# hrdkjain/GenIcoNet

Hardware: AMD Instinct MI355X
Metric: meshes/sec training throughput, ico2ico I5 batch=36 (higher is better)
Workload: dtype f32; 1 GPU; ico2ico AE training, I5, batch 36 per GPU (BASELINE configs[1]); per_gpu_batch=36, global_batch=36, subdivisions=5, parallelism=dp1

## Files before the change

geniconet_amd/csrc/icn_api.cpp:

```cpp
#include <hip/hip_runtime.h>

#include <algorithm>
#include <cstdio>
#include <cstdlib>
#include <cstring>
#include <map>
#include <mutex>
#include <stdexcept>
#include <string>
#include <tuple>
#include <vector>

#include "../../include/icn.h"
#include "icn_geometry.h"
#include "icn_launch.h"
#include "icn_streamk.h"

namespace {

thread_local std::string g_err;

int fail(const std::string& msg) {
    g_err = msg;
    return -1;
// ... 25 lines not shown
    int32_t* code = nullptr;
    int32_t* slots = nullptr;
    int n_slots = 0, E = 1;
};
DevDma upload_dma(const std::vector<int32_t>& idx, int E, int P) {
    icn::DmaTable h;
    icn::build_dma_table(idx, E, P, h);
    DevDma d;
    d.code = upload(h.code);
    d.slots = upload(h.slots);
    d.n_slots = h.n_slots;
    d.E = E;
    return d;
}
struct ConvTables {
    int Pin = 0, Pout = 0, n_in = 0, n_out = 0, E = 1;
    int32_t* fwd = nullptr;
    int32_t* bwd = nullptr;
    int32_t* bwd1 = nullptr;
    int nv = 0, nvp = 0;
    int32_t* vidx = nullptr;
    int32_t* vorder = nullptr;
    uint32_t* vmask32 = nullptr;
    int32_t* vq = nullptr;
    int32_t* perm = nullptr;
    int32_t* bwd_perm = nullptr;
    uint32_t* mask32 = nullptr;
    std::vector<uint32_t> mask32_h;
    int key = 0;
    DevDma d_fwd, d_bwd, d_bwd1, d_virt, d_bwdp;
    int32_t* w7_rows = nullptr;
    uint16_t* w7_pos = nullptr;
    int w7_U = 0;
};
struct UpTables {
    int Pc = 0, Pf = 0, Wf = 0, Wb = 0;
    int32_t *idx_f = nullptr, *idx_b = nullptr;
    float *coef_f = nullptr, *coef_b = nullptr;
};

struct UpconvDev {
    int Pc = 0, Pf = 0, n_slots = 0, E = 1, nseg = 0;
    int seg_cnt[icn::UPCONV_MAX_SEG] = {}, seg_off[icn::UPCONV_MAX_SEG] = {};
    uint32_t seg_mask[icn::UPCONV_MAX_SEG] = {};
    int32_t *pix = nullptr, *code = nullptr, *slot_idx = nullptr;
    float *alpha = nullptr, *slot_coef = nullptr;
};

struct EllSplitDev {
    int W = 0, n_ovf = 0, W_ovf = 0;
    int32_t *idx = nullptr, *ovf_rows = nullptr, *ovf_idx = nullptr;
    float *coef = nullptr, *ovf_coef = nullptr;
};
EllSplitDev upload_ell_split(const icn::Ell& e, int W_main) {
    EllSplitDev d;
    const int W = e.width;
    d.W = W_main;
    d.W_ovf = std::max(W - W_main, 0);
    std::vector<int32_t> idx((size_t)e.rows * W_main, icn::IDX_ZERO), ovf_rows, ovf_idx;
    std::vector<float> coef((size_t)e.rows * W_main, 0.f), ovf_coef;
    for (int r = 0; r < e.rows; ++r) {
        for (int k = 0; k < std::min(W, W_main); ++k) {
            idx[(size_t)r * W_main + k] = e.idx[(size_t)r * W + k];
            coef[(size_t)r * W_main + k] = e.coef[(size_t)r * W + k];
        }
        if (W > W_main && e.idx[(size_t)r * W + W_main] != icn::IDX_ZERO) {
            ovf_rows.push_back(r);
            for (int k = W_main; k < W; ++k) {
                ovf_idx.push_back(e.idx[(size_t)r * W + k]);
                ovf_coef.push_back(e.coef[(size_t)r * W + k]);
            }
        }
    }
    d.n_ovf = (int)ovf_rows.size();
    d.idx = upload(idx);
    d.coef = upload(coef);
    d.ovf_rows = upload(ovf_rows);
    d.ovf_idx = upload(ovf_idx);
    d.ovf_coef = upload(ovf_coef);
    return d;
}

struct PatchHost { std::vector<int32_t> prow; std::vector<uint16_t> plocal; int npatch = 0, umax = 0, gridW = 0; };
bool build_patches(const std::vector<int32_t>& idx, int width_in, int width, int H, int W, int ph, int pw, PatchHost& out) {
    out = PatchHost{};
    if (H % ph != 0 || W % pw != 0 || (long)H * W * width_in != (long)idx.size()) return false;
    const int pr_n = H / ph, pc_n = W / pw;
    out.npatch = pr_n * pc_n;
    out.gridW = W;
    out.plocal.assign((size_t)H * W * width, 0xFFFFu);
    std::vector<std::vector<int32_t>> lists(out.npatch);
    for (int p = 0; p < out.npatch; ++p) {
        std::vector<int32_t>& u = lists[p];
        for (int i = 0; i < ph; ++i)
            for (int j = 0; j < pw; ++j) {
                const size_t r = (size_t)((p / pc_n) * ph + i) * W + (p % pc_n) * pw + j;
                for (int k = 0; k < width; ++k) {
                    const int32_t v = idx[r * width_in + k];
                    if (v >= 0) u.push_back(v);
                }
            }
        std::sort(u.begin(), u.end());
        u.erase(std::unique(u.begin(), u.end()), u.end());
        out.umax = std::max(out.umax, (int)u.size());
    }
    out.umax = (out.umax + 31) / 32 * 32;
    if (out.umax == 0 || out.umax >= 0xFFFF) return false;
    out.prow.assign((size_t)out.npatch * out.umax, -1);
    for (int p = 0; p < out.npatch; ++p) {
        const std::vector<int32_t>& u = lists[p];
        std::copy(u.begin(), u.end(), out.prow.begin() + (size_t)p * out.umax);
        for (int i = 0; i < ph; ++i)
            for (int j = 0; j < pw; ++j) {
                const size_t r = (size_t)((p / pc_n) * ph + i) * W + (p % pc_n) * pw + j;
                for (int k = 0; k < width; ++k) {
                    const int32_t v = idx[r * width_in + k];
                    if (v >= 0) out.plocal[r * width + k] = (uint16_t)(std::lower_bound(u.begin(), u.end(), v) - u.begin());
                }
            }
    }
    return true;
}
struct PatchDev { int32_t* prow = nullptr; uint16_t* plocal = nullptr; int npatch = 0, umax = 0, gridW = 0; };
PatchDev upload_patches(const PatchHost& h) {
    PatchDev d;
    if (getenv("ICN_VERBOSE")) fprintf(stderr, "icn: patch table: %d patches, %d rows per list, grid width %d\n", h.npatch, h.umax, h.gridW);
    d.prow = upload(h.prow);
    d.plocal = upload(h.plocal);
    d.npatch = h.npatch; d.umax = h.umax; d.gridW = h.gridW;
    return d;
}

struct UpconvBwdDev {
    int Pc = 0, Pf = 0;
    PatchDev sc_patch, ga_patch;
    EllSplitDev gather, scatter;
    int32_t* iota = nullptr;
    int32_t* px_srcs = nullptr;
    int32_t* px_cls = nullptr;
    float* cls_coef = nullptr;
    int n_cls = 0;
};

std::mutex g_mu;
std::map<std::tuple<int, int, int>, UpconvDev> g_upconv;
std::map<std::tuple<int, int, int>, UpconvBwdDev> g_upconv_bwd;
std::map<std::tuple<int, int, int, int>, ConvTables> g_conv;
std::map<std::tuple<int, int, int>, UpTables> g_up;

static int wgrad7_union_rows(int stride) {
    if (stride != 1) return 112;
    static const int u1 = [] {
        const char* e = getenv("ICN_W7_U");
        return e ? atoi(e) : 64;
    }();
    if (u1 != 56 && u1 != 64)
        throw std::invalid_argument("icn: ICN_W7_U must be 56 or 64 (the instantiations of k_wgrad7 at stride 1), got " + std::to_string(u1));
    return u1;
}

ConvTables make_conv_tables(int r_in, int stride, int mode) {
    ConvTables t;
    t.n_in = 1 << r_in;
    t.n_out = t.n_in / stride;
    t.Pin = icn::pixels(r_in);
    t.Pout = 10 * t.n_out * t.n_out;
    std::vector<int32_t> fwd, bwd, perm;
    std::vector<uint8_t> mask;
    icn::build_conv_fwd(r_in, stride, mode, fwd);
    t.E = icn::build_conv_bwd(r_in, stride, mode, bwd);
    t.fwd = upload(fwd);
    t.bwd = upload(bwd);
    t.d_fwd = upload_dma(fwd, 1, t.Pout);
    t.d_bwd = upload_dma(bwd, t.E, t.Pin);
    {
        icn::DmaTable h;
        icn::build_dma_table(fwd, 1, t.Pout, h);
        icn::Wg7Table w7;
        if (icn::build_wgrad7(h, t.Pout, wgrad7_union_rows(stride), w7)) {
            t.w7_rows = upload(w7.urow);
            t.w7_pos = upload(w7.upos);
            t.w7_U = w7.U;
        }
    }
    std::vector<int32_t> primary;
    icn::VirtualRows vr;
    icn::split_conv_bwd(r_in, stride, bwd, t.E, primary, vr);
    t.bwd1 = upload(primary);
    t.d_bwd1 = upload_dma(primary, 1, t.Pin);
    t.nv = vr.nv;
    if (vr.nv > 0) {
        std::vector<int32_t> order, vidx_o;
        std::vector<uint8_t> vmask;
        icn::build_virtual_order(vr, t.nvp, order, vidx_o, vmask);
        t.vidx = upload(vidx_o);
        t.vorder = upload(order);
        t.vmask32 = upload(std::vector<uint32_t>(vmask.begin(), vmask.end()));
        t.d_virt = upload_dma(vidx_o, 1, t.nvp);
        t.vq = upload(vr.vq);
    }
// ... 85 lines not shown
UpconvBwdDev make_upconv_bwd_tables(int r_in, int mode) {
    icn::Ell e, f;
    icn::build_upconv_bwd(r_in, mode, e);
    icn::build_upconv_scatter(r_in, mode, f);
    UpconvBwdDev d;
    d.Pc = icn::pixels(r_in);
    d.Pf = 4 * d.Pc;
    {
        constexpr int NS = 20;
        std::vector<int32_t> srcs((size_t)d.Pc * NS, icn::IDX_ZERO);
        std::vector<float> coefd((size_t)d.Pc * NS * 8, 0.f);
        icn::Ell rest;
        rest.width = e.width;
        std::vector<int32_t> rest_rows;
        for (int sp = 0; sp < d.Pc; ++sp) {
            std::vector<int32_t> uniq;
            for (int t = 0; t < 7; ++t)
                for (int k = 0; k < e.width; ++k) {
                    const int32_t p = e.idx[((size_t)sp * 7 + t) * e.width + k];
                    if (p >= 0 && std::find(uniq.begin(), uniq.end(), p) == uniq.end()) uniq.push_back(p);
                }
            if ((int)uniq.size() <= NS) {
                std::sort(uniq.begin(), uniq.end());
                for (size_t k = 0; k < uniq.size(); ++k) srcs[(size_t)sp * NS + k] = uniq[k];
                for (int t = 0; t < 7; ++t)
                    for (int k = 0; k < e.width; ++k) {
                        const int32_t p = e.idx[((size_t)sp * 7 + t) * e.width + k];
                        if (p < 0) continue;
                        const size_t slot = std::lower_bound(uniq.begin(), uniq.end(), p) - uniq.begin();
                        coefd[((size_t)sp * NS + slot) * 8 + t] += e.coef[((size_t)sp * 7 + t) * e.width + k];
                    }
            } else {
                for (int t = 0; t < 7; ++t) {
                    rest_rows.push_back(sp * 7 + t);
                    rest.idx.insert(rest.idx.end(), e.idx.begin() + ((size_t)sp * 7 + t) * e.width, e.idx.begin() + ((size_t)sp * 7 + t + 1) * e.width);
                    rest.coef.insert(rest.coef.end(), e.coef.begin() + ((size_t)sp * 7 + t) * e.width, e.coef.begin() + ((size_t)sp * 7 + t + 1) * e.width);
                }
            }
        }
        rest.rows = (int)rest_rows.size();
        std::vector<int32_t> cls(d.Pc, 0);
        std::vector<float> cls_coef(NS * 8, 0.f);
        std::map<std::vector<float>, int> seen;
        seen.emplace(std::vector<float>(NS * 8, 0.f), 0);
        for (int sp = 0; sp < d.Pc; ++sp) {
            std::vector<float> blk(coefd.begin() + (size_t)sp * NS * 8, coefd.begin() + (size_t)(sp + 1) * NS * 8);
            auto found = seen.find(blk);
            if (found == seen.end()) {
                if ((int)seen.size() >= icn::UPCONV_PX_CLASSES) {
                    for (int k = 0; k < NS; ++k) srcs[(size_t)sp * NS + k] = icn::IDX_ZERO;
                    for (int t = 0; t < 7; ++t) {
                        rest_rows.push_back(sp * 7 + t);
                        rest.idx.insert(rest.idx.end(), e.idx.begin() + ((size_t)sp * 7 + t) * e.width, e.idx.begin() + ((size_t)sp * 7 + t + 1) * e.width);
                        rest.coef.insert(rest.coef.end(), e.coef.begin() + ((size_t)sp * 7 + t) * e.width, e.coef.begin() + ((size_t)sp * 7 + t + 1) * e.width);
                    }
                    continue;
                }
                found = seen.emplace(blk, (int)seen.size()).first;
                cls_coef.insert(cls_coef.end(), blk.begin(), blk.end());
            }
            cls[sp] = found->second;
        }
        rest.rows = (int)rest_rows.size();
        d.n_cls = (int)seen.size();
        d.px_srcs = upload(srcs);
        {
            const int n = 1 << r_in;
            PatchHost ph;
            if (build_patches(srcs, NS, NS, 5 * n, 2 * n, 4, 8, ph)) d.ga_patch = upload_patches(ph);
        }
        d.px_cls = upload(cls);
        d.cls_coef = upload(cls_coef);
        d.gather = EllSplitDev{};
        d.gather.n_ovf = rest.rows;
        d.gather.W_ovf = rest.width;
        d.gather.ovf_rows = upload(rest_rows);
        d.gather.ovf_idx = upload(rest.idx);
        d.gather.ovf_coef = upload(rest.coef);
    }
    d.scatter = upload_ell_split(f, 16);
    {
        const int n = 1 << r_in;
        PatchHost ph;
        if (f.width >= 1 && build_patches(f.idx, f.width, std::min(f.width, 16), 10 * n, 4 * n, 8, 16, ph) && std::min(f.width, 16) == 16)
            d.sc_patch = upload_patches(ph);
    }
    std::vector<int32_t> iota(d.Pc);
    for (int i = 0; i < d.Pc; ++i) iota[i] = i;
    d.iota = upload(iota);
    return d;
}
const UpconvBwdDev& upconv_bwd_tables(int r_in, int mode) {
    int dev = 0;
    ICN_HIP(hipGetDevice(&dev));
    std::lock_guard<std::mutex> lk(g_mu);
    auto key = std::make_tuple(dev, r_in, mode);
    auto it = g_upconv_bwd.find(key);
    if (it != g_upconv_bwd.end()) return it->second;
    return g_upconv_bwd.emplace(key, make_upconv_bwd_tables(r_in, mode)).first->second;
}

int upconv_slots(int r_in) {
    static std::mutex mu;
    static std::map<int, int> cache;
    std::lock_guard<std::mutex> lk(mu);
    auto it = cache.find(r_in);
    if (it != cache.end()) return it->second;
    int n = 0;
    for (int mode = 0; mode < 2; ++mode) {
        icn::UpconvTable h;
        icn::build_upconv_fwd(r_in, mode, h);
        n = std::max(n, h.n_slots);
    }
    return cache[r_in] = n;
}

struct ProfRec { int kind; double flops; hipEvent_t e0, e1; };
std::vector<ProfRec> g_prof;
size_t g_prof_used = 0;
bool g_prof_on = false, g_prof_open = false;
int g_prof_only = -1;
std::mutex g_prof_mu;

void check_conv(const void* a, const void* b, const void* c, int B, int Cin, int Cout, int r_in, int stride) {
    if (!a || !b || !c) throw std::invalid_argument("icn: null tensor pointer");
    if (B < 1 || Cin < 1 || Cout < 1) throw std::invalid_argument("icn: B, Cin, Cout must be positive");
    if (r_in < 0 || r_in > 10) throw std::invalid_argument("icn: subdivisions out of range [0,10]");
    if (stride != 1 && stride != 2) throw std::invalid_argument("icn: stride must be 1 or 2");
    if ((size_t)B * icn::pixels(r_in) >= (size_t)1 << 31) throw std::invalid_argument("icn: B * pixels exceeds int32 rows");
}

inline size_t align256(size_t x) { return (x + 255) & ~(size_t)255; }

struct TableCounts { int nv = 0, slots_fwd = 0, slots_bwd = 0; };
TableCounts table_counts(int r_in, int stride) {
    static std::mutex mu;
    static std::map<std::pair<int, int>, TableCounts> cache;
    std::lock_guard<std::mutex> lk(mu);
    auto key = std::make_pair(r_in, stride);
    auto it = cache.find(key);
    if (it != cache.end()) return it->second;
    TableCounts c;
    const int Pin = icn::pixels(r_in), Pout = Pin / (stride * stride);
    for (int mode = 0; mode < 2; ++mode) {
        std::vector<int32_t> fwd, bwd, primary;
        icn::DmaTable d;
        icn::build_conv_fwd(r_in, stride, mode, fwd);
        icn::build_dma_table(fwd, 1, Pout, d);
        c.slots_fwd = std::max(c.slots_fwd, d.n_slots);
        const int E = icn::build_conv_bwd(r_in, stride, mode, bwd);
        icn::build_dma_table(bwd, E, Pin, d);
        c.slots_bwd = std::max(c.slots_bwd, d.n_slots);
        if (stride == 1) {
            icn::VirtualRows vr;
            icn::split_conv_bwd(r_in, 1, bwd, E, primary, vr);
            c.nv = std::max(c.nv, (vr.nv + 31) / 32 * 32);
            if (vr.nv > 0) {
                icn::build_dma_table(vr.vidx, 1, vr.nv, d);
                c.slots_bwd = std::max(c.slots_bwd, d.n_slots);
            }
        }
    }
    return cache[key] = c;
}

size_t wgrad_partial_bytes(int M, int Cin, int Cout, int Cout0) {
    return align256((size_t)icn::wgrad_splits(M, Cin, Cout, Cout0) * 7 * Cin * Cout * sizeof(float));
// ... 1172 lines not shown
```

geniconet_amd/csrc/icn_kernels.hip:

```cpp
#include <hip/hip_runtime.h>
#include <stdint.h>

#include <algorithm>
#include <cfloat>
#include <atomic>
#include <cstdio>
#include <cstdlib>
#include <cstring>
#include <map>
#include <mutex>
#include <tuple>
#include <vector>
#include <stdexcept>
#include <type_traits>
#include <utility>

#include "icn_launch.h"
#include "icn_streamk.h"

#ifndef ICN_CHAIN_PRIO
#define ICN_CHAIN_PRIO 0
#endif
#if ICN_CHAIN_PRIO > 0
#define ICN_CHAIN_SETPRIO() __builtin_amdgcn_s_setprio(ICN_CHAIN_PRIO)
// ... 2278 lines not shown
            float v[8];
#pragma unroll
            for (int u = 0; u < 8; ++u) v[u] = k + u < k1 ? src[(size_t)(k + u) * stride] : 0.f;
            s0 += v[0] + v[4];
            s1 += v[1] + v[5];
            s2 += v[2] + v[6];
            s3 += v[3] + v[7];
        }
    }
    red[q][lane] = (s0 + s1) + (s2 + s3);
    __syncthreads();
    if (q == 0) {
        const float v = (red[0][lane] + red[1][lane]) + (red[2][lane] + red[3][lane]);
        if (is_w) {
            const int co = i % Cout, ci = (i / Cout) % Cin, t = i / (Cin * Cout);
            if (co < Cout0) dw[((size_t)co * Cin + ci) * 7 + t] = v;
            else dw2[((size_t)(co - Cout0) * Cin + ci) * 7 + t] = v;
        } else if (is_b) {
            const int co = i - total;
            if (co < Cout0) { if (dbias) dbias[co] = v; }
            else if (dbias2) dbias2[co - Cout0] = v;
        }
    }
}

__global__ void k_wgrad_generic(const float* __restrict__ x, const float* __restrict__ dy, const int32_t* __restrict__ idx,
                                float* __restrict__ partial, float* __restrict__ bias_partial, int M, int Ps, int Pd, int Cin,
                                int Cout, int ns, int rows_per_split) {
    const int total = 7 * Cin * Cout;
    const int m0 = blockIdx.y * rows_per_split, m1 = min(M, m0 + rows_per_split);
    for (int i = blockIdx.x * blockDim.x + threadIdx.x; i < total; i += gridDim.x * blockDim.x) {
        const int co = i % Cout, ci = (i / Cout) % Cin, t = i / (Cin * Cout);
        const bool do_bias = bias_partial != nullptr && t == 0 && ci == 0;
        float s = 0.f, sb = 0.f;
        for (int m = m0; m < m1; ++m) {
            const int b = m / Pd, p = m % Pd;
            const float dyv = dy[(size_t)m * Cout + co];
            if (do_bias) sb += dyv;
            const int32_t code = idx[(size_t)t * Pd + p];
            if (code == -1) continue;
            s += gather1(x, code, b, Ps, ns, Cin, ci) * dyv;
        }
        partial[(size_t)blockIdx.y * total + i] = s;
        if (do_bias) bias_partial[(size_t)blockIdx.y * Cout + co] = sb;
    }
}

constexpr int STEM_PIX = 64;
constexpr int STEM_WG_PIX = 256;

template <int CIN, int NPIX = STEM_PIX>
__device__ __forceinline__ void stem_gather(const float* __restrict__ x, const int32_t* __restrict__ idx, float* xs, int m0,
                                            int M, int Ps, int Pd, int ns) {
    for (int i = threadIdx.x; i < NPIX * 7; i += 256) {
        const int row = i / 7, t = i % 7, m = m0 + row;
        float v[CIN];
#pragma unroll
        for (int ci = 0; ci < CIN; ++ci) v[ci] = 0.f;
        if (m < M) {
            const int b = m / Pd, p = m % Pd;
            const int32_t code = idx[(size_t)t * Pd + p];
#pragma unroll
            for (int ci = 0; ci < CIN; ++ci) v[ci] = gather1(x, code, b, Ps, ns, CIN, ci);
        }
#pragma unroll
        for (int ci = 0; ci < CIN; ++ci) xs[row * (7 * CIN) + t * CIN + ci] = v[ci];
    }
}

template <int CIN>
__global__ __launch_bounds__(256) void k_stem_fwd(const float* __restrict__ x, const float* __restrict__ w,
                                                   const float* __restrict__ bias, float* __restrict__ y,
                                                   const int32_t* __restrict__ idx, int M, int Ps, int Pd, int Cout, int ns) {
    constexpr int KT = 7 * CIN;
    extern __shared__ __attribute__((aligned(16))) char smem[];
    float* w_s = reinterpret_cast<float*>(smem);
    float* b_s = w_s + KT * Cout;
    float* xs = b_s + Cout;
    for (int i = threadIdx.x; i < KT * Cout; i += 256) {
        const int co = i % Cout, k = i / Cout, ci = k % CIN, t = k / CIN;
        w_s[i] = w[((size_t)co * CIN + ci) * 7 + t];
    }
    for (int i = threadIdx.x; i < Cout; i += 256) b_s[i] = bias ? bias[i] : 0.f;
    const int q = Cout / 4;
    for (int m0 = blockIdx.x * STEM_PIX; m0 < M; m0 += gridDim.x * STEM_PIX) {
        __syncthreads();
        stem_gather<CIN>(x, idx, xs, m0, M, Ps, Pd, ns);
        __syncthreads();
        for (int i = threadIdx.x; i < STEM_PIX * q; i += 256) {
            const int row = i / q, c4 = (i % q) * 4, m = m0 + row;
            if (m >= M) continue;
            f32x4 acc = *reinterpret_cast<const f32x4*>(b_s + c4);
#pragma unroll
            for (int k = 0; k < KT; ++k) acc += xs[row * KT + k] * *reinterpret_cast<const f32x4*>(w_s + k * Cout + c4);
            *reinterpret_cast<f32x4*>(y + (size_t)m * Cout + c4) = acc;
        }
    }
}

template <int CIN>
__global__ __launch_bounds__(256) void k_stem_wgrad(const float* __restrict__ x, const float* __restrict__ dy,
                                                     const int32_t* __restrict__ idx, float* __restrict__ partial,
                                                     float* __restrict__ bias_partial, int M, int Ps, int Pd, int Cout, int ns,
                                                     int rows_per_block) {
    constexpr int KT = 7 * CIN, NA = KT + 1;
    extern __shared__ __attribute__((aligned(16))) char smem[];
    float* xs = reinterpret_cast<float*>(smem);
    f32x4* red = reinterpret_cast<f32x4*>(smem);
    const int q = Cout / 4, G = 256 / q, g = threadIdx.x / q, c4 = threadIdx.x % q;
    const int mb = blockIdx.x * rows_per_block, me = min(M, mb + rows_per_block);
    f32x4 acc[NA];
#pragma unroll
    for (int i = 0; i < NA; ++i) acc[i] = f32x4{0.f, 0.f, 0.f, 0.f};
    for (int mg = mb; mg < me; mg += STEM_WG_PIX) {
        __syncthreads();
        stem_gather<CIN, STEM_WG_PIX>(x, idx, xs, mg, me, Ps, Pd, ns);
        __syncthreads();
        for (int m0 = mg; m0 < min(me, mg + STEM_WG_PIX); m0 += STEM_PIX) {
            const float* xg = xs + (m0 - mg) * KT;
            const int nrow = min(STEM_PIX, me - m0);
            f32x4 dyv[4];
#pragma unroll
            for (int u = 0; u < 4; ++u) {
                const int row = g + u * G;
                dyv[u] = (row < nrow && u * G < STEM_PIX) ? ld4(dy + (size_t)(m0 + row) * Cout + 4 * c4) : f32x4{0.f, 0.f, 0.f, 0.f};
            }
#pragma unroll
            for (int u = 0; u < 4; ++u) {
                const int row = g + u * G;
                if (row >= nrow || u * G >= STEM_PIX) break;
                acc[KT] += dyv[u];
#pragma unroll
                for (int k = 0; k < KT; ++k) acc[k] += dyv[u] * xg[row * KT + k];
            }
            for (int row = g + 4 * G; row < nrow; row += G) {
                const f32x4 d = ld4(dy + (size_t)(m0 + row) * Cout + 4 * c4);
                acc[KT] += d;
#pragma unroll
                for (int k = 0; k < KT; ++k) acc[k] += d * xg[row * KT + k];
            }
        }
    }
    __syncthreads();
    const int lane = threadIdx.x & 63, wave = threadIdx.x >> 6, wq = q < 64 ? q : 64;
#pragma unroll
    for (int i = 0; i < NA; ++i)
        for (int off = wq; off < 64; off <<= 1)
#pragma unroll
            for (int e = 0; e < 4; ++e) acc[i][e] += __shfl_xor(acc[i][e], off, 64);
    const int nwv = q <= 64 ? 4 : 256 / q;
    if (lane < wq) {
#pragma unroll
        for (int i = 0; i < NA; ++i) red[((q <= 64 ? wave : g) * NA + i) * q + c4] = acc[i];
    }
    __syncthreads();
    for (int i = threadIdx.x; i < NA * q; i += 256) {
        f32x4 s = {0.f, 0.f, 0.f, 0.f};
        for (int k = 0; k < nwv; ++k) s += red[k * NA * q + i];
        const int a = i / q, c = (i % q) * 4;
        if (a < KT) *reinterpret_cast<f32x4*>(partial + ((size_t)blockIdx.x * KT + a) * Cout + c) = s;
        else if (bias_partial) *reinterpret_cast<f32x4*>(bias_partial + (size_t)blockIdx.x * Cout + c) = s;
    }
}

bool stem_supported(int Cin, int Cout) { return Cin >= 1 && Cin <= 4 && Cout >= 4 && Cout <= 256 && 256 % Cout == 0; }

void launch_stem_fwd(const float* x, const float* w, const float* bias, float* y, const int32_t* idx, int M, int Ps, int Pd,
                     int Cin, int Cout, int ns, hipStream_t s) {
    const int blocks = std::min(4096, (M + STEM_PIX - 1) / STEM_PIX);
    const size_t lds = ((size_t)(7 * Cin + 1) * Cout + (size_t)STEM_PIX * 7 * Cin) * 4;
#define ICN_SF(C) hipLaunchKernelGGL((k_stem_fwd<C>), dim3(blocks), dim3(256), lds, s, x, w, bias, y, idx, M, Ps, Pd, Cout, ns)
    switch (Cin) { case 1: ICN_SF(1); break; case 2: ICN_SF(2); break; case 3: ICN_SF(3); break; default: ICN_SF(4); }
#undef ICN_SF
}

bool wgrad_supported(int Cin, int Cout) { return Cin % 64 == 0 && Cout % 64 == 0; }

// ... 241 lines not shown

__global__ __launch_bounds__(256) void k_upconv_gather(const float* __restrict__ dy0, const float* __restrict__ dy1,
                                                        float* __restrict__ g, const int32_t* __restrict__ idx,
                                                        const float* __restrict__ coef, const int32_t* __restrict__ rows, int B,
                                                        int Pin, int nrows, int rows_total, int C0, int C1, int W, int acc) {
    const int C = C0 + C1, cv = C / 4;
    const size_t total = (size_t)B * nrows * cv;
    for (size_t i = (size_t)blockIdx.x * blockDim.x + threadIdx.x; i < total; i += (size_t)gridDim.x * blockDim.x) {
        const int c = (int)(i % cv) * 4;
        const size_t br = i / cv;
        const int r = (int)(br % nrows), b = (int)(br / nrows);
        const bool second = c >= C0;
        const float* src = (second ? dy1 : dy0) + (size_t)b * Pin * (second ? C1 : C0) + (second ? c - C0 : c);
        const int stride = second ? C1 : C0;
        f32x4 sum = {0.f, 0.f, 0.f, 0.f};
        for (int e0 = 0; e0 < W; e0 += 8) {
            int32_t j[8];
            float w[8];
#pragma unroll
            for (int k = 0; k < 8; ++k) {
                const bool in_row = e0 + k < W;
                j[k] = in_row ? idx[(size_t)r * W + e0 + k] : -1;
                w[k] = in_row ? coef[(size_t)r * W + e0 + k] : 0.f;
            }
            f32x4 x[8];
#pragma unroll
            for (int k = 0; k < 8; ++k) x[k] = j[k] >= 0 ? ld4(src + (size_t)j[k] * stride) : f32x4{0.f, 0.f, 0.f, 0.f};
#pragma unroll
            for (int k = 0; k < 8; ++k) sum += w[k] * x[k];
        }
        float* o = g + ((size_t)b * rows_total + (rows ? rows[r] : r)) * C + c;
        if (acc) sum += ld4(o);
        *reinterpret_cast<f32x4*>(o) = sum;
    }
}

__global__ __launch_bounds__(256) void k_upconv_scatter(const float* __restrict__ z, const float* __restrict__ bias,
                                                         float* __restrict__ y0, float* __restrict__ y1,
                                                         const int32_t* __restrict__ idx, const float* __restrict__ coef,
                                                         const int32_t* __restrict__ rows, int B, int zrows, int nrows, int Pout,
                                                         int C0, int C1, int W, int acc) {
    const int C = C0 + C1, cv = C / 4;
    for (XcdWalk w_((size_t)B * nrows * cv); w_.pos < w_.end; w_.pos += w_.step) {
        const size_t i = w_.pos;
        const int c = (int)(i % cv) * 4;
        const size_t br = i / cv;
        const int r = (int)(br % nrows), b = (int)(br / nrows);
        const float* src = z + (size_t)b * zrows * C + c;
        f32x4 sum = {0.f, 0.f, 0.f, 0.f};
        if (bias && !acc) sum = ld4(bias + c);
        for (int e0 = 0; e0 < W; e0 += 8) {
            int32_t j[8];
            float w[8];
#pragma unroll
            for (int k = 0; k < 8; ++k) {
                const bool in_row = e0 + k < W;
                j[k] = in_row ? idx[(size_t)r * W + e0 + k] : -1;
                w[k] = in_row ? coef[(size_t)r * W + e0 + k] : 0.f;
            }
            f32x4 x[8];
#pragma unroll
            for (int k = 0; k < 8; ++k) x[k] = j[k] >= 0 ? ld4(src + (size_t)j[k] * C) : f32x4{0.f, 0.f, 0.f, 0.f};
#pragma unroll
            for (int k = 0; k < 8; ++k) sum += w[k] * x[k];
        }
        const int row = rows ? rows[r] : r;
        float* o = c < C0 ? y0 + ((size_t)b * Pout + row) * C0 + c : y1 + ((size_t)b * Pout + row) * C1 + (c - C0);
        if (acc) sum += ld4(o);
        *reinterpret_cast<f32x4*>(o) = sum;
    }
}

void launch_upconv_scatter(const float* z, const float* bias, float* y0, float* y1, const int32_t* idx, const float* coef,
                           const int32_t* rows, int B, int zrows, int nrows, int Pout, int C0, int C1, int W, int acc, hipStream_t s) {
    if (nrows <= 0) return;
    const size_t total = (size_t)B * nrows * ((C0 + C1) / 4);
    hipLaunchKernelGGL(k_upconv_scatter, dim3(xcd_grid(total, 16384)), dim3(256), 0, s, z, bias, y0, y1,
                       idx, coef, rows, B, zrows, nrows, Pout, C0, C1, W, acc);
}

constexpr int PATCH_CH = 32;
constexpr int PATCH_IT_MAX = 14;

__device__ __forceinline__ void patch_stage(const float* __restrict__ src, unsigned src_bytes, const int32_t* __restrict__ prow_l,
                                            int n_it, int b, int rows_per_sample, int Cs, int c0, float* rows_s) {
#if defined(__HIP_DEVICE_COMPILE__)
    const int lane = threadIdx.x & 63, wave = __builtin_amdgcn_readfirstlane(threadIdx.x >> 6);
    const auto rsrc = __builtin_amdgcn_make_buffer_rsrc(const_cast<float*>(src), 0, src_bytes, 0x00020000);
#pragma unroll
    for (int it = 0; it < PATCH_IT_MAX; ++it) {
        if (it < n_it) {
            const int row = prow_l[it];
            const unsigned off = row >= 0 ? ((unsigned)(b * rows_per_sample + row) * (unsigned)Cs + (unsigned)c0) * 4u + 16u * (lane & 7)
                                          : 0xC0000000u;
            float* dst = rows_s + __builtin_amdgcn_readfirstlane((it * 32 + wave * 8) * PATCH_CH);
            __builtin_amdgcn_raw_ptr_buffer_load_lds(rsrc, (lds_ptr_t)dst, 16, off, 0, 0, 0);
        }
    }
#endif
}

constexpr int PS_W = 16;
constexpr int PS_PH = 8, PS_PW = 16;
__global__ __launch_bounds__(256, 3) void k_upconv_scatter_lds(const float* __restrict__ z, const float* __restrict__ bias,
                                                             float* __restrict__ y0, float* __restrict__ y1,
                                                             const int32_t* __restrict__ prow, const uint16_t* __restrict__ plocal,
                                                             const float* __restrict__ coef, int B, int zrows, int Pout, int C0,
                                                             int C1, int npatch, int umax, int gridW, int bgroup, int cgroup,
                                                             unsigned z_bytes) {
#if defined(__HIP_DEVICE_COMPILE__)
    extern __shared__ __attribute__((aligned(16))) char smem[];
    float* rows_s = reinterpret_cast<float*>(smem);
    const int C = C0 + C1, nchunk = C / PATCH_CH, n_it = umax / 32;
    const int nbg = (B + bgroup - 1) / bgroup, ncg = (nchunk + cgroup - 1) / cgroup, items = npatch * nbg * ncg;
    const int per = (items + 7) / 8, item = (blockIdx.x % 8) * per + blockIdx.x / 8;
    if (blockIdx.x / 8 >= per || item >= items) return;
    const int patch = item % npatch, bg = (item / npatch) % nbg, cg = item / (npatch * nbg);
    const int ch_end = min(nchunk, (cg + 1) * cgroup);
    const int ppr = gridW / PS_PW;
    const int tid = threadIdx.x, lane = tid & 63, wave = tid >> 6;
    const int px = tid >> 1, half = tid & 1;
    const int orow = ((patch / ppr) * PS_PH + px / PS_PW) * gridW + (patch % ppr) * PS_PW + px % PS_PW;
    int li[PS_W];
    float cf[PS_W];
    {
        const uint16_t* lp = plocal + (size_t)orow * PS_W;
        const float* cp = coef + (size_t)orow * PS_W;
#pragma unroll
        for (int e = 0; e < PS_W; ++e) {
            const unsigned v = lp[e];
            li[e] = (v == 0xFFFFu ? umax : (int)v) * PATCH_CH + half * 16;
            cf[e] = v == 0xFFFFu ? 0.f : cp[e];
        }
    }
    if (tid < PATCH_CH) rows_s[umax * PATCH_CH + tid] = 0.f;
    int32_t prow_l[PATCH_IT_MAX];
#pragma unroll
    for (int it = 0; it < PATCH_IT_MAX; ++it)
        prow_l[it] = it < n_it ? prow[(size_t)patch * umax + it * 32 + wave * 8 + (lane >> 3)] : -1;
    const int b_end = min(B, (bg + 1) * bgroup);
    for (int b = bg * bgroup; b < b_end; ++b)
        for (int ch = cg * cgroup; ch < ch_end; ++ch) {
            const int c0 = ch * PATCH_CH;
            patch_stage(z, z_bytes, prow_l, n_it, b, zrows, C, c0, rows_s);
            asm volatile("s_waitcnt vmcnt(0)" ::: "memory");
            __syncthreads();
            const int c = c0 + half * 16;
            f32x4 acc[4];
#pragma unroll
            for (int q = 0; q < 4; ++q) acc[q] = bias ? ld4(bias + c + 4 * q) : f32x4{0.f, 0.f, 0.f, 0.f};
#pragma unroll
            for (int e = 0; e < PS_W; ++e) {
                const float* r = rows_s + li[e];
#pragma unroll
                for (int q = 0; q < 4; ++q) acc[q] += cf[e] * ld4(r + 4 * q);
            }
            float* o = c < C0 ? y0 + ((size_t)b * Pout + orow) * C0 + c : y1 + ((size_t)b * Pout + orow) * C1 + (c - C0);
#pragma unroll
            for (int q = 0; q < 4; ++q) *reinterpret_cast<f32x4*>(o + 4 * q) = acc[q];
            __syncthreads();
        }
#endif
}

static void patch_groups(int npatch, int B, int nchunk, int& bgroup, int& cgroup) {
    const long passes = (long)npatch * B * nchunk;
    long per = passes / (4L * 768);
    per = per < 4 ? 4 : (per > 16 ? 16 : per);
    cgroup = (int)std::min<long>(nchunk, per);
    bgroup = (int)std::max<long>(1, per / cgroup);
}

void launch_upconv_scatter_lds(const float* z, const float* bias, float* y0, float* y1, const PatchTab& t, const float* coef, int B,
                               int zrows, int Pout, int C0, int C1, hipStream_t s) {
    int bgroup, cgroup;
    patch_groups(t.npatch, B, (C0 + C1) / PATCH_CH, bgroup, cgroup);
    const int items = t.npatch * ((B + bgroup - 1) / bgroup) * (((C0 + C1) / PATCH_CH + cgroup - 1) / cgroup);
    const int grid = (items + 7) / 8 * 8;
    const size_t lds = (size_t)(t.umax + 1) * PATCH_CH * 4;
    static std::atomic<uint64_t> attr_devices{0};
    if (!((attr_devices.load(std::memory_order_relaxed) >> current_device_bit()) & 1)) {
        (void)hipFuncSetAttribute(reinterpret_cast<const void*>(&k_upconv_scatter_lds), hipFuncAttributeMaxDynamicSharedMemorySize, 64 * 1024);
        attr_devices.fetch_or((uint64_t)1 << current_device_bit(), std::memory_order_relaxed);
    }
    hipLaunchKernelGGL(k_upconv_scatter_lds, dim3(grid), dim3(256), lds, s, z, bias, y0, y1, t.prow, t.plocal, coef, B, zrows, Pout, C0,
                       C1, t.npatch, t.umax, t.gridW, bgroup, cgroup, (unsigned)((size_t)B * zrows * (C0 + C1) * 4));
}
bool upconv_patch_usable(const PatchTab& t, int B, size_t rows_per_sample, int C0, int C1) {
    if (dbg_flags() & 1024) return false;
    if (t.prow == nullptr || t.umax < 32 || t.umax > 32 * PATCH_IT_MAX || t.umax % 32) return false;
    if (C0 % PATCH_CH || C1 % PATCH_CH) return false;
    return (size_t)B * rows_per_sample * std::max(C0 + C1, 1) * 4 < ((size_t)3 << 30);
}

constexpr int PG_PH = 4, PG_PW = 8;
__global__ __launch_bounds__(256, 3) void k_upconv_gather_lds(const float* __restrict__ dy0, const float* __restrict__ dy1,
                                                            float* __restrict__ g, const int32_t* __restrict__ prow,
                                                            const uint16_t* __restrict__ plocal, const int32_t* __restrict__ cls,
                                                            const float* __restrict__ cls_coef, int ncls, int B, int Pin, int Pc,
                                                            int C0, int C1, int npatch, int umax, int gridW, int bgroup, int cgroup) {
#if defined(__HIP_DEVICE_COMPILE__)
    extern __shared__ __attribute__((aligned(16))) char smem[];
    f32x4* ctab = reinterpret_cast<f32x4*>(smem);
    float* rows_s = reinterpret_cast<float*>(ctab + ncls * 20 * 2);
    for (int i = threadIdx.x; i < ncls * 20 * 2; i += 256) ctab[i] = ld4(cls_coef + 4 * i);
    const int C = C0 + C1, nchunk = C / PATCH_CH, n_it = umax / 32;
    const int nbg = (B + bgroup - 1) / bgroup, ncg = (nchunk + cgroup - 1) / cgroup, items = npatch * nbg * ncg;
    const int per = (items + 7) / 8, item = (blockIdx.x % 8) * per + blockIdx.x / 8;
    if (blockIdx.x / 8 >= per || item >= items) return;
    const int patch = item % npatch, bg = (item / npatch) % nbg, cg = item / (npatch * nbg);
    const int ch_end = min(nchunk, (cg + 1) * cgroup);
    const int ppr = gridW / PG_PW;
    const int tid = threadIdx.x, lane = tid & 63, wave = tid >> 6;
    const int px = tid >> 3, q = tid & 7;
    const int sp = ((patch / ppr) * PG_PH + px / PG_PW) * gridW + (patch % ppr) * PG_PW + px % PG_PW;
    int li[20];
    {
        const uint16_t* lp = plocal + (size_t)sp * 20;
#pragma unroll
        for (int k = 0; k < 20; ++k) { const unsigned v = lp[k]; li[k] = (v == 0xFFFFu ? umax : (int)v) * PATCH_CH + 4 * q; }
    }
    if (tid < PATCH_CH) rows_s[umax * PATCH_CH + tid] = 0.f;
    const f32x4* cf = ctab + cls[sp] * 40;
    int32_t prow_l[PATCH_IT_MAX];
#pragma unroll
    for (int it = 0; it < PATCH_IT_MAX; ++it)
        prow_l[it] = it < n_it ? prow[(size_t)patch * umax + it * 32 + wave * 8 + (lane >> 3)] : -1;
    const unsigned b0_bytes = (unsigned)((size_t)B * Pin * C0 * 4), b1_bytes = (unsigned)((size_t)B * Pin * C1 * 4);
    const int b_end = min(B, (bg + 1) * bgroup);
    __syncthreads();
    for (int b = bg * bgroup; b < b_end; ++b)
        for (int ch = cg * cgroup; ch < ch_end; ++ch) {
            const int c0 = ch * PATCH_CH;
            if (c0 < C0) patch_stage(dy0, b0_bytes, prow_l, n_it, b, Pin, C0, c0, rows_s);
            else patch_stage(dy1, b1_bytes, prow_l, n_it, b, Pin, C1, c0 - C0, rows_s);
            asm volatile("s_waitcnt vmcnt(0)" ::: "memory");
            __syncthreads();
            f32x4 acc[7];
// ... 201 lines not shown
```

Baseline: 5678 meshes/s.

## Swizzle LDS patch rows, reorder patch lists tap-major, hoist stem weights

```diff
diff --git a/geniconet_amd/csrc/icn_api.cpp b/geniconet_amd/csrc/icn_api.cpp
--- a/geniconet_amd/csrc/icn_api.cpp
+++ b/geniconet_amd/csrc/icn_api.cpp
@@ -131,7 +131,8 @@
 }
 
 struct PatchHost { std::vector<int32_t> prow; std::vector<uint16_t> plocal; int npatch = 0, umax = 0, gridW = 0; };
-bool build_patches(const std::vector<int32_t>& idx, int width_in, int width, int H, int W, int ph, int pw, PatchHost& out) {
+bool build_patches(const std::vector<int32_t>& idx, int width_in, int width, int H, int W, int ph, int pw, PatchHost& out,
+                   int tap_major_w = 0) {
     out = PatchHost{};
     if (H % ph != 0 || W % pw != 0 || (long)H * W * width_in != (long)idx.size()) return false;
     const int pr_n = H / ph, pc_n = W / pw;
@@ -156,15 +157,27 @@
     out.umax = (out.umax + 31) / 32 * 32;
     if (out.umax == 0 || out.umax >= 0xFFFF) return false;
     out.prow.assign((size_t)out.npatch * out.umax, -1);
+    std::vector<uint16_t> pos;
     for (int p = 0; p < out.npatch; ++p) {
         const std::vector<int32_t>& u = lists[p];
-        std::copy(u.begin(), u.end(), out.prow.begin() + (size_t)p * out.umax);
+        pos.resize(u.size());
+        for (size_t k = 0; k < u.size(); ++k) pos[k] = (uint16_t)k;
+        if (tap_major_w > 0) {
+            std::vector<uint16_t> order(pos);
+            auto key = [&](uint16_t k) {
+                const int32_t s = u[k] / 7, t = u[k] % 7;
+                return std::make_tuple(s / tap_major_w, t, s % tap_major_w);
+            };
+            std::sort(order.begin(), order.end(), [&](uint16_t a, uint16_t b) { return key(a) < key(b); });
+            for (size_t k = 0; k < order.size(); ++k) pos[order[k]] = (uint16_t)k;
+        }
+        for (size_t k = 0; k < u.size(); ++k) out.prow[(size_t)p * out.umax + pos[k]] = u[k];
         for (int i = 0; i < ph; ++i)
             for (int j = 0; j < pw; ++j) {
                 const size_t r = (size_t)((p / pc_n) * ph + i) * W + (p % pc_n) * pw + j;
                 for (int k = 0; k < width; ++k) {
                     const int32_t v = idx[r * width_in + k];
-                    if (v >= 0) out.plocal[r * width + k] = (uint16_t)(std::lower_bound(u.begin(), u.end(), v) - u.begin());
+                    if (v >= 0) out.plocal[r * width + k] = pos[std::lower_bound(u.begin(), u.end(), v) - u.begin()];
                 }
             }
     }
@@ -416,7 +429,7 @@
     {
         const int n = 1 << r_in;
         PatchHost ph;
-        if (f.width >= 1 && build_patches(f.idx, f.width, std::min(f.width, 16), 10 * n, 4 * n, 8, 16, ph) && std::min(f.width, 16) == 16)
+        if (f.width >= 1 && build_patches(f.idx, f.width, std::min(f.width, 16), 10 * n, 4 * n, 8, 16, ph, 2 * n) && std::min(f.width, 16) == 16)
             d.sc_patch = upload_patches(ph);
     }
     std::vector<int32_t> iota(d.Pc);
diff --git a/geniconet_amd/csrc/icn_kernels.hip b/geniconet_amd/csrc/icn_kernels.hip
--- a/geniconet_amd/csrc/icn_kernels.hip
+++ b/geniconet_amd/csrc/icn_kernels.hip
@@ -2384,17 +2384,22 @@
         w_s[i] = w[((size_t)co * CIN + ci) * 7 + t];
     }
     for (int i = threadIdx.x; i < Cout; i += 256) b_s[i] = bias ? bias[i] : 0.f;
-    const int q = Cout / 4;
+    const int q = Cout / 4, c4 = (threadIdx.x % q) * 4, row0 = threadIdx.x / q, rstep = 256 / q;
+    __syncthreads();
+    f32x4 wr[KT];
+#pragma unroll
+    for (int k = 0; k < KT; ++k) wr[k] = *reinterpret_cast<const f32x4*>(w_s + k * Cout + c4);
+    const f32x4 br = *reinterpret_cast<const f32x4*>(b_s + c4);
     for (int m0 = blockIdx.x * STEM_PIX; m0 < M; m0 += gridDim.x * STEM_PIX) {
         __syncthreads();
         stem_gather<CIN>(x, idx, xs, m0, M, Ps, Pd, ns);
         __syncthreads();
-        for (int i = threadIdx.x; i < STEM_PIX * q; i += 256) {
-            const int row = i / q, c4 = (i % q) * 4, m = m0 + row;
-            if (m >= M) continue;
-            f32x4 acc = *reinterpret_cast<const f32x4*>(b_s + c4);
-#pragma unroll
-            for (int k = 0; k < KT; ++k) acc += xs[row * KT + k] * *reinterpret_cast<const f32x4*>(w_s + k * Cout + c4);
+        for (int row = row0; row < STEM_PIX; row += rstep) {
+            const int m = m0 + row;
+            if (m >= M) break;
+            f32x4 acc = br;
+#pragma unroll
+            for (int k = 0; k < KT; ++k) acc += xs[row * KT + k] * wr[k];
             *reinterpret_cast<f32x4*>(y + (size_t)m * Cout + c4) = acc;
         }
     }
@@ -2802,6 +2807,7 @@
 constexpr int PATCH_CH = 32;
 constexpr int PATCH_IT_MAX = 14;
 
+template <bool SWZ = false>
 __device__ __forceinline__ void patch_stage(const float* __restrict__ src, unsigned src_bytes, const int32_t* __restrict__ prow_l,
                                             int n_it, int b, int rows_per_sample, int Cs, int c0, float* rows_s) {
 #if defined(__HIP_DEVICE_COMPILE__)
@@ -2811,7 +2817,8 @@
     for (int it = 0; it < PATCH_IT_MAX; ++it) {
         if (it < n_it) {
             const int row = prow_l[it];
-            const unsigned off = row >= 0 ? ((unsigned)(b * rows_per_sample + row) * (unsigned)Cs + (unsigned)c0) * 4u + 16u * (lane & 7)
+            const unsigned chunk = SWZ ? (unsigned)((lane & 7) ^ ((lane >> 4) & 3)) : (unsigned)(lane & 7);
+            const unsigned off = row >= 0 ? ((unsigned)(b * rows_per_sample + row) * (unsigned)Cs + (unsigned)c0) * 4u + 16u * chunk
                                           : 0xC0000000u;
             float* dst = rows_s + __builtin_amdgcn_readfirstlane((it * 32 + wave * 8) * PATCH_CH);
             __builtin_amdgcn_raw_ptr_buffer_load_lds(rsrc, (lds_ptr_t)dst, 16, off, 0, 0, 0);
@@ -2839,17 +2846,20 @@
     const int ch_end = min(nchunk, (cg + 1) * cgroup);
     const int ppr = gridW / PS_PW;
     const int tid = threadIdx.x, lane = tid & 63, wave = tid >> 6;
-    const int px = tid >> 1, half = tid & 1;
-    const int orow = ((patch / ppr) * PS_PH + px / PS_PW) * gridW + (patch % ppr) * PS_PW + px % PS_PW;
-    int li[PS_W];
+    const int half = lane & 1, slot = (lane >> 1) & 15;
+    const unsigned odd = (0xC33Cu >> slot) & 1u;
+    const int k = __popc((odd ? 0xC33Cu : 0x3CC3u) & ((1u << slot) - 1u));
+    const int pi = wave * 2 + (lane >> 5), pj = 2 * k + (int)odd;
+    const int orow = ((patch / ppr) * PS_PH + pi) * gridW + (patch % ppr) * PS_PW + pj;
+    unsigned li[PS_W];
     float cf[PS_W];
     {
         const uint16_t* lp = plocal + (size_t)orow * PS_W;
         const float* cp = coef + (size_t)orow * PS_W;
 #pragma unroll
         for (int e = 0; e < PS_W; ++e) {
-            const unsigned v = lp[e];
-            li[e] = (v == 0xFFFFu ? umax : (int)v) * PATCH_CH + half * 16;
+            const unsigned v = lp[e], u = v == 0xFFFFu ? (unsigned)umax : v;
+            li[e] = u * (PATCH_CH * 4) + half * 64 + (((u >> 1) & 3u) << 4);
             cf[e] = v == 0xFFFFu ? 0.f : cp[e];
         }
     }
@@ -2862,18 +2872,20 @@
     for (int b = bg * bgroup; b < b_end; ++b)
         for (int ch = cg * cgroup; ch < ch_end; ++ch) {
             const int c0 = ch * PATCH_CH;
-            patch_stage(z, z_bytes, prow_l, n_it, b, zrows, C, c0, rows_s);
+            patch_stage<true>(z, z_bytes, prow_l, n_it, b, zrows, C, c0, rows_s);
             asm volatile("s_waitcnt vmcnt(0)" ::: "memory");
             __syncthreads();
             const int c = c0 + half * 16;
             f32x4 acc[4];
 #pragma unroll
             for (int q = 0; q < 4; ++q) acc[q] = bias ? ld4(bias + c + 4 * q) : f32x4{0.f, 0.f, 0.f, 0.f};
+            unsigned qm[4] = {0u, 16u, 32u, 48u};
+            asm volatile("" : "+v"(qm[1]), "+v"(qm[2]), "+v"(qm[3]));
 #pragma unroll
             for (int e = 0; e < PS_W; ++e) {
-                const float* r = rows_s + li[e];
-#pragma unroll
-                for (int q = 0; q < 4; ++q) acc[q] += cf[e] * ld4(r + 4 * q);
+#pragma unroll
+                for (int q = 0; q < 4; ++q)
+                    acc[q] += cf[e] * *reinterpret_cast<const f32x4*>(smem + (q ? li[e] ^ qm[q] : li[e]));
             }
             float* o = c < C0 ? y0 + ((size_t)b * Pout + orow) * C0 + c : y1 + ((size_t)b * Pout + orow) * C1 + (c - C0);
 #pragma unroll
```

New measurement: 5672 meshes/s. No clear change (-0.1%).
